# sloisel/MultiGridBarrier.jl

Measured on NVIDIA B200. Metric: mgb_solve DOF*Newton-steps/s (fem2d_P1 ~1.6M DOF, p=1.5), higher is better.
Workload: dtype f64

## Files before the change

multigridbarrier.jl_b200/build.py:

```python
from __future__ import annotations

import os
import shutil
import subprocess
import sys
from concurrent.futures import ThreadPoolExecutor

HERE = os.path.dirname(os.path.abspath(__file__))
CSRC = os.path.join(HERE, "csrc")
OBJ = os.path.join(HERE, "build")
LIB = os.path.join(HERE, "libmgbx.so")
HDR = os.path.join("..", "..", "include", "mgbx.h")
ENGINE = ["engine.hpp", "host_sparse.hpp", "device_common.cuh", "node_barrier.cuh", "pcg2.hpp", HDR]
SOURCES = {
    "mgbx.cu": ["mgbx.cu", "host_amg.hpp"] + ENGINE,
    "setup.cu": ["setup.cu", "setup_kernels.cuh"] + ENGINE,
    "evaluate.cu": ["evaluate.cu", "kernels.cuh", "dense_kernels.cuh"] + ENGINE,
    "linear_solve.cu": ["linear_solve.cu", "solver_kernels.cuh"] + ENGINE,
    "newton.cu": ["newton.cu"] + ENGINE,
    "pcg2.cu": ["pcg2.cu", "pcg2.hpp"],
}
FLAGS = ["-gencode", "arch=compute_100a,code=sm_100a", "-O3", "-DNDEBUG", "-lineinfo", "-std=c++17",
         "-Xcompiler", "-fPIC,-O2,-Wall,-Wno-unused-function"]


def nvcc_path():
    for c in (os.environ.get("NVCC"), shutil.which("nvcc"), "/usr/local/cuda/bin/nvcc"):
        if c and os.path.exists(c):
            return c
    raise RuntimeError("nvcc not found")


def _obj(src):
    return os.path.join(OBJ, os.path.splitext(src)[0] + ".o")


def _stale(src):
    o = _obj(src)
    if not os.path.exists(o):
        return True
    t = os.path.getmtime(o)
    return any(os.path.getmtime(os.path.join(CSRC, d)) > t for d in SOURCES[src])


def needs_build():
    if not os.path.exists(LIB):
        return True
    t = os.path.getmtime(LIB)
    return any(_stale(s) or os.path.getmtime(_obj(s)) > t for s in SOURCES)


def _compile(src, verbose):
    cmd = [nvcc_path()] + FLAGS + (["-Xptxas", "-v"] if verbose else []) + ["-c", os.path.join(CSRC, src), "-o", _obj(src)]
# ... 27 lines not shown
```

multigridbarrier.jl_b200/csrc/device_common.cuh:

```cuda
#pragma once
#include <cuda_runtime.h>
#include <stdint.h>

#include "node_barrier.cuh"

namespace mgbx {

#define MGBX_MAX_OPS 8
constexpr int kRedBlocks = 592;
constexpr int kRedThreads = 256;

struct DevCsr {
  int64_t rows = 0, cols = 0, nnz = 0;
  int64_t *ptr = nullptr;
  int32_t *idx = nullptr;
  double *val = nullptr;
};

__device__ __forceinline__ double warp_sum(double v) {
#pragma unroll
  for (int o = 16; o > 0; o >>= 1) v += __shfl_down_sync(0xffffffffu, v, o);
  return v;
}
__device__ __forceinline__ double warp_max(double v) {
// ... 249 lines not shown
}
__device__ __forceinline__ void fence_proxy_async_smem() { asm volatile("fence.proxy.async.shared::cta;" ::: "memory"); }

struct SellPlan {
  int64_t nout = 0, nslices = 0, nterms = 0;
  int64_t *sptr = nullptr;
  int32_t *cnt = nullptr;
  int32_t *src = nullptr;
  double *w = nullptr;
};

__device__ __forceinline__ int64_t csr_find(const DevCsr &A, int64_t row, int32_t col) {
  int64_t lo = A.ptr[row], hi = A.ptr[row + 1];
  while (lo < hi) {
    const int64_t mid = (lo + hi) >> 1;
    const int32_t c = A.idx[mid];
    if (c < col) lo = mid + 1;
    else if (c > col) hi = mid;
    else return mid;
  }
  return -1;
}

constexpr int kCoarseMaxDense = 128;
inline size_t coarse_inverse_smem(int m) { return sizeof(double) * ((size_t)m * (m + 1) + (size_t)m * (m + 1) / 2 + m); }
inline size_t dense_solve_small_smem(int m) { return sizeof(double) * ((size_t)m * (m + 1) + 2 * (size_t)m); }

constexpr int kGemmBM = 64, kGemmBN = 64, kGemmBK = 16, kGemmLd = kGemmBK + 4;

__device__ __forceinline__ void dmma_m8n8k4(double &d0, double &d1, double a, double b) {
  asm volatile("mma.sync.aligned.m8n8k4.row.col.f64.f64.f64.f64 {%0,%1}, {%2}, {%3}, {%0,%1};" : "+d"(d0), "+d"(d1) : "d"(a), "d"(b));
}

constexpr int kCholNB = 64;
constexpr size_t kCholDiagSmem = sizeof(double) * 2 * kCholNB * (kCholNB + 1);

struct KronCombo {
  const double *Qj, *Qk;
  const double *h;
};
constexpr int kKronMaxCombos = 16;
struct KronWArgs {
  int n1, c2a, c2b, ncombo, K;
  KronCombo c[kKronMaxCombos];
};

struct TopPlanParams {
  DevCsr R;
  DevCsr EincT;
  DevCsr pat;
  const int32_t *rowof;
  int64_t n, N;
  int p, nkept, unit;
  int kept[MGBX_MAX_ND];
  int64_t off[MGBX_MAX_ND + 1];
  int64_t rcol0[MGBX_MAX_ND];
  int pair_of[MGBX_MAX_ND * MGBX_MAX_ND];
};

}
```

multigridbarrier.jl_b200/csrc/engine.hpp:

```cpp
#pragma once
#include <cuda_runtime.h>

#include <chrono>
#include <cmath>
#include <cstdio>
#include <cstring>
#include <functional>
#include <map>
#include <memory>
#include <string>
#include <vector>

#include "host_sparse.hpp"
#include "device_common.cuh"
#include "pcg2.hpp"

namespace mgbx {

#define CK(call)                                                                                      \
  do {                                                                                                \
    cudaError_t e_ = (call);                                                                          \
    if (e_ != cudaSuccess)                                                                            \
      throw std::runtime_error(std::string("CUDA error: ") + cudaGetErrorString(e_) + " at " + __FILE__ + ":" + \
                               std::to_string(__LINE__));                                             \
// ... 182 lines not shown
};

struct EvalOut {
  double y, gnorm;
  bool finite;
  double nonfinite_nodes, lin;
};

}

struct mgbx_handle {
  mgbx::Pool pool;
  mgbx::Amg amg[2];
  std::string err;
  mgbx_config cfg;
  cudaStream_t stream = nullptr;
  bool has_feas = false;
  double *partials = nullptr;
  unsigned int *ticket = nullptr;
  double *dscal = nullptr;
  double *hscal = nullptr;
  mgbx_step_result *res = nullptr;
  int64_t launches = 0;
  int64_t kc_launches[mgbx::KC_COUNT] = {0};
  double kc_ms[mgbx::KC_COUNT] = {0};
  std::vector<cudaEvent_t> ev_free;
  struct Pending {
    int kc;
    cudaEvent_t a, b;
  };
  std::vector<Pending> ev_pending;
  cudaEvent_t ev_cur = nullptr;
  int pcg2_grid = 0;
  double dgemm_flops = 0.0;
  double cur_rtol2 = 1e-22;
  int cur_window = 25;
  int rank = 0, nranks = 1;
  void *comm = nullptr;
  int device = -1;
  std::vector<double> prof_ns;
  std::vector<int64_t> prof_cnt;
  std::vector<unsigned long long> prof_host;
};
namespace mgbx {

struct SolveResult {
  int iters = 0;
  int status = 1;
  double rel = 0.0;
  double erel = 0.0;
};

struct Engine {
  mgbx_handle *h;
  cudaStream_t s;
  explicit Engine(mgbx_handle *hh) : h(hh), s(hh->stream) {}

  void sync() {
    CK(cudaStreamSynchronize(s));
    if (!h->ev_pending.empty()) {
      for (auto &p : h->ev_pending) {
        float ms = 0.f;
        cudaEventElapsedTime(&ms, p.a, p.b);
        if (p.kc >= 0) h->kc_ms[p.kc] += ms;
        else if (h->res) {
          if (p.kc == STAGE_F01) h->res->ms_f01 += ms;
// ... 67 lines not shown
  static int group_for(const DevCsr &A) {
    const double avg = A.rows ? (double)A.nnz / (double)A.rows : 0.0;
    return avg > 48.0 ? 32 : (avg > 6.0 ? 4 : 1);
  }
  void spmv(const DevCsr &A, const double *x, const double *y0, double alpha, double *y, int G = 0);
  void axpby(int64_t m, double a, const double *x, double b, const double *y, double *out);
  void prolong_to_fine(Amg &A, int J, const double *x, const double *zbase, double *zf);
  void restrict_from_fine(Amg &A, int J, const double *gb, double *gJ);
  void dot2_fetch(Amg &A, int J, const double *a, const double *b);
  void maxabs_fetch(int64_t n, const double *v);
  void trial(Amg &A, int J, double sigma);
  void phase1_slack(Amg &A, Amg &F);
  void blockgrad(Amg &A, const ElemParams &E);
  NodeParams node_params(Amg &A, double t);
  ElemParams elem_params(Amg &A);
  bool elem_fused_setup(Amg &A, const NodeParams &NP, int nex, ElemFused &Q, size_t &smem, unsigned int &grid);
  int plap_dim(const Amg &A) const;
  bool plap_setup(Amg &A, int dim, double t, bool use_bw, PlapParams &Q, size_t &smem, unsigned int &grid, bool cond = true);
  EvalOut eval_f01(Amg &A, int J, double t, const double *zbase, const double *x, double *gout, bool use_bw = true);

  System &system_for(Amg &A, int J);
  void assemble(Amg &A, System &S, int J, double t, const double *zbase, const double *x);
  void assemble_unfused(Amg &A, System &S, int J, double t, const double *x);
  void galerkin(System &S, int kend);
  void schur_masks(const Amg &A, const System &S, unsigned &pieces, unsigned &elim) const;
  void assemble_dense(Amg &A, System &S, const NodeParams &P);
  void dgemm_nt(int M, int N, int K, const double *Am, int64_t lda, const double *Bm, int64_t ldb, const double *sc, double *C, int64_t ldc, bool acc, double alpha = 1.0);

  bool precond_fp32(const System &S) const;
  int lambda_power_its(const System &S) const;
  bool use_direct(const System &S, const SysLevel &Lv) const;
  std::vector<int> active_levels(const System &S, int ktop) const;
  void setup_hierarchy(Amg &A, System &S, int ktop);
  void dense_factor(SysLevel &Lv);
  void dense_apply(SysLevel &Lv, const double *b, double *x);
  void direct_solve(SysLevel &Lv, const double *b, double *x);
  SellBuild make_sell(const DevCsr &A, int64_t nthreads);
  void sell_prepare(System &S, int ktop);
  System::Pcg2Dev &pcg2_plan(System &S, int ktop);
  void pcg2_setup_dist(System::Pcg2Dev &D, int nshard);
  SolveResult pcg(System &S, int ktop, const double *b, double *x);
  SolveResult solve_compact(System &S, int ktop, const double *b, double *x);
  SolveResult solve(Amg &A, System &S, int J, const double *g, double *dir);

  struct NewtonOut {
    bool converged;
    int k;
    int status;
    double y, gnorm, inc;
  };
  NewtonOut newton(Amg &A, int J, double t, int maxit, int stop_kind, double lambda_tol, double theta, const mgbx_step_opts &o);
  int step(int which, double t, const mgbx_step_opts &o, mgbx_step_result *r);
  int matched_t(double t_default, double *t_out, double *tstar_out);
};

void solve_kernels_init();
void kron_w_init(size_t smem);

inline bool dense_mode(const Amg &A) { return A.N == 1 && A.p > 64; }
constexpr int kDenseMaxUnknowns = 8192;

template <class F>
bool kron_factor(F M, int r1, int r2, int c1, int c2, std::vector<double> &A, std::vector<double> &B) {
  const int64_t rows = (int64_t)r1 * r2, cols = (int64_t)c1 * c2;
  double best = 0.0;
  int64_t pr = 0, pc = 0;
  for (int64_t r = 0; r < rows; ++r)
    for (int64_t c = 0; c < cols; ++c) {
      const double v = std::fabs(M(r, c));
      if (v > best) {
        best = v;
        pr = r;
        pc = c;
      }
    }
  if (!(best > 0.0) || !std::isfinite(best)) return false;
  const int a0 = (int)(pr / r2), b0 = (int)(pr % r2), g0 = (int)(pc / c2), d0 = (int)(pc % c2);
  A.assign((size_t)r1 * c1, 0.0);
  B.assign((size_t)r2 * c2, 0.0);
  for (int b = 0; b < r2; ++b)
    for (int d = 0; d < c2; ++d) B[(size_t)b * c2 + d] = M((int64_t)a0 * r2 + b, (int64_t)g0 * c2 + d);
  const double piv = B[(size_t)b0 * c2 + d0];
  for (int a = 0; a < r1; ++a)
    for (int g = 0; g < c1; ++g) A[(size_t)a * c1 + g] = M((int64_t)a * r2 + b0, (int64_t)g * c2 + d0) / piv;
  const double tol = 1e-12 * best;
  for (int64_t r = 0; r < rows; ++r)
    for (int64_t c = 0; c < cols; ++c)
      if (std::fabs(M(r, c) - A[(size_t)(r / r2) * c1 + (c / c2)] * B[(size_t)(r % r2) * c2 + (c % c2)]) > tol) return false;
  return true;
// ... 13 lines not shown
```

multigridbarrier.jl_b200/csrc/linear_solve.cu:

```cuda
#include "engine.hpp"
#include "solver_kernels.cuh"

namespace mgbx {

void solve_kernels_init() {
  CK(cudaFuncSetAttribute(k_coarse_inverse, cudaFuncAttributeMaxDynamicSharedMemorySize, (int)coarse_inverse_smem(kCoarseMaxDense)));
  CK(cudaFuncSetAttribute(k_dense_solve_small, cudaFuncAttributeMaxDynamicSharedMemorySize, (int)dense_solve_small_smem(kCoarseMaxDense)));
  CK(cudaFuncSetAttribute(k_chol_diag_inv, cudaFuncAttributeMaxDynamicSharedMemorySize, (int)kCholDiagSmem));
  CK(cudaFuncSetAttribute(k_chol_solve_blocked, cudaFuncAttributeMaxDynamicSharedMemorySize, (int)(sizeof(double) * kDenseMaxUnknowns)));
}

bool Engine::precond_fp32(const System &S) const {
  if (h->cfg.precond_fp32 != 2) return h->cfg.precond_fp32 == 1;
  int64_t tot = 0;
  for (const SysLevel &Lv : S.lev) tot += Lv.A.nnz;
  return tot >= 10000000;
}
int Engine::lambda_power_its(const System &S) const {
  if (h->cfg.lambda_power >= 0) return h->cfg.lambda_power;
  if (S.lev.empty() || S.lev[0].A.rows == 0) return 0;
  return ((double)S.lev[0].A.nnz / (double)S.lev[0].A.rows > 16.0) ? 6 : 0;
}
bool Engine::use_direct(const System &S, const SysLevel &Lv) const {
  return S.dense || Lv.m <= h->cfg.dense_direct_max;
}
std::vector<int> Engine::active_levels(const System &S, int ktop) const {
  const int nlev = (int)S.lev.size();
  const int kend = (S.cut >= 0) ? std::max(S.cut, ktop) : nlev - 1;
  std::vector<int> act;
  for (int k = ktop; k <= kend; ++k) {
    if (k < kend && S.lev[k].T_identity) continue;
    act.push_back(k);
  }
  return act;
}

void Engine::setup_hierarchy(Amg &A, System &S, int ktop) {
  const int nlev = (int)S.lev.size();
  SysLevel &Ltop = S.lev[ktop];
  const bool direct = use_direct(S, Ltop);
  int kend = ktop;
  if (!direct) kend = (S.cut >= 0) ? std::max(S.cut, ktop) : nlev - 1;
  galerkin(S, kend);
  if (direct) {
    if (Ltop.m > kCoarseMaxDense) dense_factor(Ltop);
    return;
  }
  for (int k = ktop; k <= kend; ++k) {
    SysLevel &Lv = S.lev[k];
    CK(cudaMemsetAsync(Lv.lam, 0, sizeof(double), s));
    LAUNCH(KC_VEC, k_l1diag<<<nblk(Lv.m), 256, 0, s>>>(Lv.A, Lv.dinv, Lv.diag, (unsigned long long *)Lv.lam));
    if (precond_fp32(S)) {
      if (!Lv.val32) Lv.val32 = h->pool.alloc<float>(Lv.A.nnz);
      LAUNCH(KC_VEC, k_f64_to_f32<<<nblk(Lv.A.nnz), 256, 0, s>>>(Lv.A.nnz, Lv.A.val, Lv.val32));
    }
  }
  if (S.cut >= 0 && S.cut >= ktop) {
    SysLevel &Lc = S.lev[S.cut];
    const int m = (int)Lc.m;
    if (!Lc.dense_inv) Lc.dense_inv = h->pool.alloc<double>((size_t)m * m);
    LAUNCH(KC_DENSE, k_coarse_inverse<<<1, 1024, coarse_inverse_smem(m), s>>>(Lc.A, Lc.dense_inv));
  }
  sell_prepare(S, ktop);
  if (lambda_power_its(S) > 0) {
    System::Pcg2Dev &D = pcg2_plan(S, ktop);
    if ((int64_t)D.host.nlev * h->pcg2_grid > 3 * (int64_t)kPcg2MaxGrid) throw std::runtime_error("internal: too many levels for the power-iteration kernel");
    LAUNCH(KC_VEC, CK(pcg2_lambda_power(D.dev, h->pcg2_grid, lambda_power_its(S), 1.2, s)));
  }
}

void Engine::dense_factor(SysLevel &Lv) {
  const int m = (int)Lv.m;
  if (m == 0) return;
  const int npan = (m + kCholNB - 1) / kCholNB;
  if (!Lv.dense) {
    Lv.dense = h->pool.alloc<double>((size_t)m * m);
    Lv.dscale = h->pool.alloc<double>(m);
    Lv.dense_inv = h->pool.alloc<double>((size_t)npan * kCholNB * kCholNB);
  }
  zero(Lv.dense, (int64_t)m * m);
  LAUNCH(KC_DENSE, k_dense_scale_diag<<<nblk(m), 256, 0, s>>>(Lv.A, Lv.dscale));
  LAUNCH(KC_DENSE, k_csr_to_dense<<<nblk(m), 256, 0, s>>>(Lv.A, Lv.dscale, Lv.dense));
  for (int p = 0; p < npan; ++p) {
    const int k0 = p * kCholNB, nb = std::min(kCholNB, m - k0), rem = m - k0 - nb;
    double *Li = Lv.dense_inv + (size_t)p * kCholNB * kCholNB;
    LAUNCH(KC_DENSE, k_chol_diag_inv<<<1, 1024, kCholDiagSmem, s>>>(Lv.dense, m, k0, Li));
    if (rem > 0) {
      double *A21 = Lv.dense + (size_t)(k0 + nb) * m + k0;
      dgemm_nt(rem, nb, nb, A21, m, Li, kCholNB, nullptr, A21, m, false);
      dgemm_nt(rem, rem, nb, A21, m, A21, m, nullptr, Lv.dense + (size_t)(k0 + nb) * m + k0 + nb, m, true, -1.0);
    }
  }
}

void Engine::dense_apply(SysLevel &Lv, const double *b, double *x) {
  const int m = (int)Lv.m;
  LAUNCH(KC_DENSE, k_chol_solve_blocked<<<1, 1024, sizeof(double) * m, s>>>(Lv.dense, m, Lv.dense_inv, Lv.dscale, b, x));
}

void Engine::direct_solve(SysLevel &Lv, const double *b, double *x) {
  const bool small = Lv.m <= kCoarseMaxDense;
  auto apply = [&](const double *rhs, double *out) {
    if (small) LAUNCH(KC_DENSE, k_dense_solve_small<<<1, 1024, dense_solve_small_smem((int)Lv.m), s>>>(Lv.A, rhs, out, nullptr));
    else dense_apply(Lv, rhs, out);
  };
  apply(b, x);
  spmv(Lv.A, x, b, -1.0, Lv.r, Lv.spmv_group);
  apply(Lv.r, Lv.x2);
  axpby(Lv.m, 1.0, x, 1.0, Lv.x2, x);
}

SellBuild Engine::make_sell(const DevCsr &A, int64_t nthreads) {
  SellBuild B;
  h->pool.cat = "solve kernel: sliced-ELL level matrices";
  if (A.rows >= INT32_MAX / 2) throw std::runtime_error("persistent solve kernel: a level matrix exceeds 32-bit indexing");
  int lpr = 1;
  const double avg = A.rows ? (double)A.nnz / (double)A.rows : 0.0;
  while (lpr < 32 && A.rows * (int64_t)lpr * 2 <= nthreads && avg / lpr >= 2.0) lpr *= 2;
  const int rps = 32 / lpr;
  const int nsl = (int)((A.rows + rps - 1) / rps);
  B.M.rows = (int)A.rows;
  B.M.lpr = lpr;
  B.M.nslices = nsl;
  B.M.spc = pcg2_slices_per_cta(nsl, std::max(1, h->pcg2_grid));
  if (nsl == 0) return B;
  int *width = tmp_alloc<int>(nsl, s);
  CK(sell_slice_widths(A.rows, lpr, A.ptr, width, s));
  std::vector<int> hw(nsl);
  CK(cudaMemcpyAsync(hw.data(), width, sizeof(int) * nsl, cudaMemcpyDeviceToHost, s));
  CK(cudaStreamSynchronize(s));
  tmp_free(width, s);
  std::vector<int> soff(nsl + 1, 0);
  int64_t tot = 0;
  for (int q = 0; q < nsl; ++q) {
    tot += 32 * (int64_t)hw[q];
    if (tot > INT32_MAX) throw std::runtime_error("persistent solve kernel: sliced-ELL level matrix exceeds 32-bit indexing");
    soff[q + 1] = (int)tot;
// ... 304 lines not shown
```

multigridbarrier.jl_b200/csrc/mgbx.cu:

```cuda
#include <dlfcn.h>

#include <numeric>

#include "engine.hpp"
#include "host_amg.hpp"

using namespace mgbx;

namespace {

thread_local std::string g_last_error;
const char *kKClassNames[KC_COUNT] = {"node_f01", "node_f2", "blockgrad", "blockhess", "csr_gather", "spmv", "spgemm",
                                             "vector", "condense", "dense", "pcg_persistent", "elem_f01", "elem_f2", "dgemm_dmma", "elem_generic_f01", "elem_generic_f2"};

Amg &amg_arg(mgbx_handle *h, int which, const char *prefix = "") {
  if (which < 0 || which > 1 || (which == 1 && !h->has_feas)) throw ArgError(std::string(prefix) + "no such AMG");
  return h->amg[which];
}
Amg &level_arg(mgbx_handle *h, int which, int level) {
  Amg &A = amg_arg(h, which);
  if (level < 0 || level >= A.L) throw ArgError("no such level");
  return A;
}

// ... 117 lines not shown
int mgbx_create(const mgbx_problem *prob, const mgbx_config *cfg, mgbx_handle **out) {
  if (!prob || !out) {
    g_last_error = "mgbx_create: null argument";
    return MGBX_ERR_ARG;
  }
  *out = nullptr;
  mgbx_handle *h = new mgbx_handle();
  if (cfg) h->cfg = *cfg;
  else mgbx_default_config(&h->cfg);
  if (h->cfg.dense_direct_max > kDenseMaxUnknowns) h->cfg.dense_direct_max = kDenseMaxUnknowns;
  if (h->cfg.coarse_max > kCoarseMaxDense) h->cfg.coarse_max = kCoarseMaxDense;
  if (h->cfg.coarse_max < 0) h->cfg.coarse_max = 0;
  h->cur_rtol2 = h->cfg.pcg_rtol * h->cfg.pcg_rtol;
  int rc = guarded(h, [&]() -> int {
    if (h->cfg.persistent != 2) throw ArgError("mgbx_config.persistent must be 2 (the only solve kernel)");
    int ndev = 0;
    cudaError_t e = cudaGetDeviceCount(&ndev);
    if (e != cudaSuccess || ndev == 0)
      throw std::runtime_error("CUDA device required: libmgbx has no CPU fallback (cudaGetDeviceCount: " +
                               std::string(cudaGetErrorString(e)) + ")");
    if (h->cfg.device >= 0) CK(cudaSetDevice(h->cfg.device));
    CK(cudaGetDevice(&h->device));
    CK(cudaStreamCreateWithFlags(&h->stream, cudaStreamNonBlocking));
    h->pool.stream = h->stream;
    {
      int dev = 0;
      CK(cudaGetDevice(&dev));
      cudaMemPool_t mp = nullptr;
      CK(cudaDeviceGetDefaultMemPool(&mp, dev));
      uint64_t keep = UINT64_MAX;
      CK(cudaMemPoolSetAttribute(mp, cudaMemPoolAttrReleaseThreshold, &keep));
      h->pcg2_grid = pcg2_grid(dev);
      if (h->pcg2_grid == 0) throw std::runtime_error("CUDA device cannot run the cooperative solve kernel");
      solve_kernels_init();
    }
    h->partials = h->pool.zeros<double>((size_t)kRedBlocks * 8, h->stream);
    h->ticket = h->pool.zeros<unsigned int>(4, h->stream);
    h->dscal = h->pool.zeros<double>(64, h->stream);
    CK(cudaMallocHost((void **)&h->hscal, sizeof(double) * 64));
    const mgbx_amg &a0 = prob->amg[0];
    create_amg(h, a0, h->amg[0]);
    Amg &A = h->amg[0];
    if (!prob->f_grid || !prob->g_grid) throw ArgError("f_grid / g_grid missing");
    CK(cudaMemcpyAsync(A.f, prob->f_grid, sizeof(double) * A.n * A.nD, cudaMemcpyHostToDevice, h->stream));
    CK(cudaMemcpyAsync(A.z, prob->g_grid, sizeof(double) * A.n * A.nu, cudaMemcpyHostToDevice, h->stream));
    CK(cudaMemcpyAsync(A.zinit, prob->g_grid, sizeof(double) * A.n * A.nu, cudaMemcpyHostToDevice, h->stream));
    if (prob->barrier_weights) A.bw = h->pool.upload<double>(prob->barrier_weights, A.n, h->stream);
    HostTimer tq;
    upload_convex(h, prob->Q, A.n, A.nD, A.cd);
    if (h->cfg.verbose > 0) fprintf(stderr, "[mgbx] convex set scanned + uploaded %.3fs\n", tq.lap());
    if (prob->amg[1].n > 0) attach_feasibility(h, prob->amg[1]);
    CK(cudaStreamSynchronize(h->stream));
    return MGBX_OK;
  });
  if (rc != MGBX_OK) {
    g_last_error = h->err;
    mgbx_destroy(h);
    return rc;
  }
  *out = h;
  return MGBX_OK;
}

static void *g_comm = nullptr;
static int g_comm_rank = -1, g_comm_nranks = 0;
static int g_comm_users = 0;

void mgbx_destroy(mgbx_handle *h) {
  if (!h) return;
  if (h->device >= 0) cudaSetDevice(h->device);
// ... 489 lines not shown
```

multigridbarrier.jl_b200/csrc/pcg2.cu:

```cuda
#include "pcg2.hpp"

#include <math.h>

namespace mgbx {
namespace {

__device__ __forceinline__ double warp_sum2(double v) {
#pragma unroll
  for (int o = 16; o > 0; o >>= 1) v += __shfl_down_sync(0xffffffffu, v, o);
  return v;
}

__device__ __forceinline__ void grid_barrier2(unsigned int *bar) {
  __syncthreads();
  if (threadIdx.x == 0) {
    unsigned int nb = 1;
    if (blockIdx.x == 0) nb = 0x80000000u - (gridDim.x - 1);
    unsigned int old, cur;
    asm volatile("atom.add.release.gpu.u32 %0,[%1],%2;" : "=r"(old) : "l"(bar), "r"(nb) : "memory");
    int spins = 0;
    do {
      asm volatile("ld.acquire.gpu.u32 %0,[%1];" : "=r"(cur) : "l"(bar) : "memory");
      if (++spins > 64) __nanosleep(40);
    } while (((old ^ cur) & 0x80000000u) == 0);
  }
  __syncthreads();
}

enum { PK_FIRST2 = 0, PK_PRE = 1, PK_RESID = 2, PK_RESTRICT = 3, PK_TAIL = 4, PK_PROLONG = 5, PK_POST = 6, PK_DENSE = 7, PK_RZSUM = 8, PK_MATVEC = 9,
       PK_UPDATE = 10, PK_INIT = 11 };
__device__ __forceinline__ void prof_mark(unsigned long long *prof, int tag) {
  if (prof && blockIdx.x == 0 && threadIdx.x == 0) {
    unsigned long long t;
    asm volatile("mov.u64 %0, %%globaltimer;" : "=l"(t));
    const unsigned long long n = prof[0];
    if (n + 1 < (unsigned long long)kPcg2ProfCap) {
      prof[1 + 2 * n] = (unsigned long long)tag;
      prof[2 + 2 * n] = t;
      prof[0] = n + 1;
    }
  }
}

template <bool GRID>
struct Ld {
  static __device__ __forceinline__ int i(const int *p) { return GRID ? __ldg(p) : *p; }
  static __device__ __forceinline__ double m(const double *p) { return GRID ? __ldg(p) : *p; }
  static __device__ __forceinline__ float mf(const float *p) { return GRID ? __ldg(p) : *p; }
  static __device__ __forceinline__ double v(const double *p) { return GRID ? __ldcg(p) : *p; }
};

struct XRt {
  unsigned long long epoch;
  int aborted;
};
__device__ __forceinline__ unsigned long long gtime() {
  unsigned long long t;
  asm volatile("mov.u64 %0, %%globaltimer;" : "=l"(t));
  return t;
// ... 850 lines not shown
```

multigridbarrier.jl_b200/csrc/solver_kernels.cuh:

```cuda
#pragma once

#include "device_common.cuh"

namespace mgbx {

__global__ void __launch_bounds__(256) k_condense_rhs(CondParams P, const double *__restrict__ g, double *Gt) {
  const int64_t i = (int64_t)blockIdx.x * blockDim.x + threadIdx.x;
  if (i >= P.n) return;
  double gE[4], tE[4], Hi[16];
  const int nE = P.nE;
  for (int ev = 0; ev < nE; ++ev) gE[ev] = g[P.Eoff[ev] + i];
  int q = 0;
  for (int a = 0; a < nE; ++a)
    for (int b = a; b < nE; ++b, ++q) {
      const double v = P.hEEinv[i + (int64_t)q * P.n];
      Hi[a * nE + b] = v;
      Hi[b * nE + a] = v;
    }
  for (int ev = 0; ev < nE; ++ev) {
    double s = 0.0;
    for (int ew = 0; ew < nE; ++ew) s += Hi[ev * nE + ew] * gE[ew];
    tE[ev] = s;
  }
  for (int a = 0; a < P.nK; ++a) {
// ... 23 lines not shown
      Hi[b * nE + a] = v;
    }
  for (int ev = 0; ev < nE; ++ev) {
    double s = 0.0;
    for (int ew = 0; ew < nE; ++ew) s += Hi[ev * nE + ew] * rE[ew];
    x[P.Eoff[ev] + i] = s;
  }
}

__global__ void k_pw_init(int64_t m, double *v) {
  const int64_t i = (int64_t)blockIdx.x * blockDim.x + threadIdx.x;
  if (i < m) v[i] = 1.0 + 0.5 * cos(0.7 * (double)i) + ((i & 1) ? 0.25 : -0.25);
}

__global__ void __launch_bounds__(256) k_l1diag(DevCsr A, double *dinv, double *diag, unsigned long long *lam_bits) {
  const int64_t row = (int64_t)blockIdx.x * blockDim.x + threadIdx.x;
  double ratio = 0.0;
  if (row < A.rows) {
    double s = 0.0, d = 0.0;
    for (int64_t k = A.ptr[row]; k < A.ptr[row + 1]; ++k) {
      s += fabs(A.val[k]);
      if (A.idx[k] == row) d = A.val[k];
    }
    dinv[row] = s > 0.0 ? 1.0 / s : 0.0;
    if (diag) diag[row] = d > 0.0 ? 1.0 / d : 0.0;
    if (d > 0.0 && isfinite(s)) ratio = s / d;
  }
  if (lam_bits) {
    ratio = warp_max(ratio);
    if ((threadIdx.x & 31) == 0 && ratio > 0.0) atomicMax(lam_bits, (unsigned long long)__double_as_longlong(ratio));
  }
}

__global__ void k_dense_scale_diag(DevCsr A, double *d) {
  const int64_t row = (int64_t)blockIdx.x * blockDim.x + threadIdx.x;
  if (row >= A.rows) return;
  double dg = 0.0;
  for (int64_t k = A.ptr[row]; k < A.ptr[row + 1]; ++k)
    if (A.idx[k] == row) dg = A.val[k];
  d[row] = dg > 0.0 ? 1.0 / sqrt(dg) : 1.0;
}

__global__ void k_csr_to_dense(DevCsr A, const double *d, double *Ad) {
  const int64_t row = (int64_t)blockIdx.x * blockDim.x + threadIdx.x;
  if (row >= A.rows) return;
  const double di = d[row];
  for (int64_t k = A.ptr[row]; k < A.ptr[row + 1]; ++k) Ad[row * A.rows + A.idx[k]] = A.val[k] * di * d[A.idx[k]];
}

__global__ void __launch_bounds__(256) k_dense_symv(const double *__restrict__ M, int m, const double *__restrict__ x, double *y) {
  const int row = (blockIdx.x * blockDim.x + threadIdx.x) >> 5;
  const int lane = threadIdx.x & 31;
  if (row >= m) return;
  const double *r = M + (size_t)row * m;
  double s = 0.0;
  for (int j = lane; j < m; j += 32) s += r[j] * x[j];
  s = warp_sum(s);
  if (lane == 0) y[row] = s;
}

__global__ void k_f64_to_f32(int64_t n, const double *__restrict__ a, float *__restrict__ out) {
  const int64_t i = (int64_t)blockIdx.x * blockDim.x + threadIdx.x;
  if (i < n) out[i] = (float)a[i];
}

__global__ void __launch_bounds__(1024) k_coarse_inverse(DevCsr A, double *Minv) {
  extern __shared__ double sm[];
  const int m = (int)A.rows;
  const int ld = m + 1;
  double *S = sm;
  double *Li = S + (size_t)m * ld;
  double *d = Li + (size_t)m * (m + 1) / 2;
  const int tid = threadIdx.x, nt = blockDim.x;
  for (int t = tid; t < m * ld; t += nt) S[t] = 0.0;
  __syncthreads();
  for (int row = tid; row < m; row += nt) {
    double dg = 0.0;
    for (int64_t k = A.ptr[row]; k < A.ptr[row + 1]; ++k)
      if (A.idx[k] == row) dg = A.val[k];
    d[row] = dg > 0.0 ? 1.0 / sqrt(dg) : 1.0;
  }
  __syncthreads();
// ... 132 lines not shown
      }
      if (tid == 0) {
        const double t = rhs[k];
        rhs[k] = rhs[pr];
        rhs[pr] = t;
      }
    }
    __syncthreads();
    const double pv = S[k * ld + k];
    for (int i = k + 1 + tid; i < m; i += nt) S[i * ld + k] /= pv;
    __syncthreads();
    const int rem = m - k - 1;
    for (int t = tid; t < rem * rem; t += nt) {
      const int i = k + 1 + t / rem, j = k + 1 + t % rem;
      S[i * ld + j] -= S[i * ld + k] * S[k * ld + j];
    }
    for (int i = k + 1 + tid; i < m; i += nt) rhs[i] -= S[i * ld + k] * rhs[k];
    __syncthreads();
  }
  if (tid < 32) {
    for (int k = m - 1; k >= 0; --k) {
      double sacc = 0.0;
      for (int j = k + 1 + tid; j < m; j += 32) sacc += S[k * ld + j] * rhs[j];
      sacc = warp_sum(sacc);
      if (tid == 0) rhs[k] = (rhs[k] - sacc) / S[k * ld + k];
      __syncwarp();
    }
  }
  __syncthreads();
  for (int i = tid; i < m; i += nt) x[i] = rhs[i];
  if (tid == 0 && info) info[0] = 1;
}

__global__ void __launch_bounds__(1024) k_chol_diag_inv(double *A, int m, int k0, double *Linv) {
  extern __shared__ double chol_sm[];
  double (*L)[kCholNB + 1] = reinterpret_cast<double (*)[kCholNB + 1]>(chol_sm);
  double (*Li)[kCholNB + 1] = reinterpret_cast<double (*)[kCholNB + 1]>(chol_sm + kCholNB * (kCholNB + 1));
  const int nb = min(kCholNB, m - k0);
  const int tid = threadIdx.x, nt = blockDim.x;
  for (int t = tid; t < kCholNB * kCholNB; t += nt) {
    const int i = t / kCholNB, j = t % kCholNB;
    L[i][j] = (i < nb && j <= i) ? A[(size_t)(k0 + i) * m + k0 + j] : 0.0;
    Li[i][j] = 0.0;
  }
  __syncthreads();
  for (int j = 0; j < nb; ++j) {
    if (tid == 0) L[j][j] = sqrt(L[j][j]);
    __syncthreads();
    const double pv = L[j][j];
    for (int i = j + 1 + tid; i < nb; i += nt) L[i][j] /= pv;
    __syncthreads();
    const int rem = nb - j - 1;
    for (int t = tid; t < rem * rem; t += nt) {
      const int i = j + 1 + t / rem, k = j + 1 + t % rem;
      if (k <= i) L[i][k] -= L[i][j] * L[k][j];
    }
    __syncthreads();
  }
  const int lane = tid & 31, wid = tid >> 5, nw = nt >> 5;
  for (int c = wid; c < nb; c += nw) {
    if (lane == 0) Li[c][c] = 1.0 / L[c][c];
    __syncwarp();
    for (int i = c + 1; i < nb; ++i) {
      double sacc = 0.0;
      for (int k = c + lane; k < i; k += 32) sacc += L[i][k] * Li[k][c];
      sacc = warp_sum(sacc);
      if (lane == 0) Li[i][c] = -sacc / L[i][i];
      __syncwarp();
    }
  }
  __syncthreads();
  for (int t = tid; t < kCholNB * kCholNB; t += nt) {
    const int i = t / kCholNB, j = t % kCholNB;
    if (i < nb && j <= i) A[(size_t)(k0 + i) * m + k0 + j] = L[i][j];
    Linv[t] = (i < nb && j < nb) ? Li[i][j] : 0.0;
  }
}

__global__ void __launch_bounds__(1024) k_chol_solve_blocked(const double *__restrict__ A, int m, const double *__restrict__ Linv,
                                                              const double *__restrict__ d, const double *__restrict__ b, double *x) {
  extern __shared__ double v[];
  __shared__ double blk[kCholNB];
  const int tid = threadIdx.x, nt = blockDim.x;
  for (int i = tid; i < m; i += nt) v[i] = b[i] * d[i];
  __syncthreads();
  const int npan = (m + kCholNB - 1) / kCholNB;
  for (int pnl = 0; pnl < npan; ++pnl) {
    const int k0 = pnl * kCholNB, nb = min(kCholNB, m - k0);
    const double *Li = Linv + (size_t)pnl * kCholNB * kCholNB;
    if (tid < nb) {
      double sacc = 0.0;
      for (int j = 0; j <= tid; ++j) sacc += Li[tid * kCholNB + j] * v[k0 + j];
      blk[tid] = sacc;
    }
    __syncthreads();
    if (tid < nb) v[k0 + tid] = blk[tid];
    for (int i = k0 + nb + tid; i < m; i += nt) {
      const double *row = A + (size_t)i * m + k0;
      double sacc = 0.0;
      for (int j = 0; j < nb; ++j) sacc += row[j] * blk[j];
      v[i] -= sacc;
    }
    __syncthreads();
  }
  for (int pnl = npan - 1; pnl >= 0; --pnl) {
    const int k0 = pnl * kCholNB, nb = min(kCholNB, m - k0);
    const double *Li = Linv + (size_t)pnl * kCholNB * kCholNB;
    const int lane = tid & 31, wid = tid >> 5, nw = nt >> 5;
    for (int j = wid; j < nb; j += nw) {
      double sacc = 0.0;
      for (int i = k0 + nb + lane; i < m; i += 32) sacc += A[(size_t)i * m + k0 + j] * v[i];
      sacc = warp_sum(sacc);
      if (lane == 0) blk[j] = v[k0 + j] - sacc;
    }
    __syncthreads();
    if (tid < nb) {
      double sacc = 0.0;
      for (int i = tid; i < nb; ++i) sacc += Li[i * kCholNB + tid] * blk[i];
      v[k0 + tid] = sacc;
    }
    __syncthreads();
  }
  for (int i = tid; i < m; i += nt) x[i] = v[i] * d[i];
}

}
```

Before: 508.9 million.

## Fuse dense Cholesky factor and solve into persistent cooperative kernels with grid barriers

Replaces the per-panel launch sequence for the dense coarse Cholesky (diagonal scaling, CSR-to-dense, per-panel diag inverse plus two DGEMM calls) with one cooperative kernel. It uses grid barriers, parallel panel TRSM across blocks and a DMMA-based trailing SYRK update. The triangular solve, residual SpMV and iterative-refinement second solve are likewise fused into one cooperative kernel with a retuned warp-parallel substitution. The goal is to remove many small launches and serialized single-block work, in exchange for grid-wide spin barriers and a dependence on cooperative launch support.

Result: faster. 541.7 million (median of 6 runs) (+6.5%).

```diff
diff --git a/multigridbarrier.jl_b200/build.py b/multigridbarrier.jl_b200/build.py
--- a/multigridbarrier.jl_b200/build.py
+++ b/multigridbarrier.jl_b200/build.py
@@ -18,7 +18,7 @@
     "evaluate.cu": ["evaluate.cu", "kernels.cuh", "dense_kernels.cuh"] + ENGINE,
     "linear_solve.cu": ["linear_solve.cu", "solver_kernels.cuh"] + ENGINE,
     "newton.cu": ["newton.cu"] + ENGINE,
-    "pcg2.cu": ["pcg2.cu", "pcg2.hpp"],
+    "pcg2.cu": ["pcg2.cu", "pcg2.hpp", "device_common.cuh", "node_barrier.cuh", HDR],
 }
 FLAGS = ["-gencode", "arch=compute_100a,code=sm_100a", "-O3", "-DNDEBUG", "-lineinfo", "-std=c++17",
          "-Xcompiler", "-fPIC,-O2,-Wall,-Wno-unused-function"]
diff --git a/multigridbarrier.jl_b200/csrc/device_common.cuh b/multigridbarrier.jl_b200/csrc/device_common.cuh
--- a/multigridbarrier.jl_b200/csrc/device_common.cuh
+++ b/multigridbarrier.jl_b200/csrc/device_common.cuh
@@ -305,8 +305,37 @@
   asm volatile("mma.sync.aligned.m8n8k4.row.col.f64.f64.f64.f64 {%0,%1}, {%2}, {%3}, {%0,%1};" : "+d"(d0), "+d"(d1) : "d"(a), "d"(b));
 }
 
+__device__ __forceinline__ void grid_barrier2(unsigned int *bar) {
+  __syncthreads();
+  if (threadIdx.x == 0) {
+    unsigned int nb = 1;
+    if (blockIdx.x == 0) nb = 0x80000000u - (gridDim.x - 1);
+    unsigned int old, cur;
+    asm volatile("atom.add.release.gpu.u32 %0,[%1],%2;" : "=r"(old) : "l"(bar), "r"(nb) : "memory");
+    int spins = 0;
+    do {
+      asm volatile("ld.acquire.gpu.u32 %0,[%1];" : "=r"(cur) : "l"(bar) : "memory");
+      if (++spins > 64) __nanosleep(40);
+    } while (((old ^ cur) & 0x80000000u) == 0);
+  }
+  __syncthreads();
+}
+
 constexpr int kCholNB = 64;
-constexpr size_t kCholDiagSmem = sizeof(double) * 2 * kCholNB * (kCholNB + 1);
+constexpr int kCholThreads = 256;
+constexpr int kCholSolveThreads = 1024;
+constexpr int kCholLd = kCholNB + 1;
+constexpr int kCholTileLd = kCholNB + 4;
+constexpr size_t kCholFactorSmem = sizeof(double) * 2 * kCholNB * kCholTileLd;
+inline size_t chol_solve_smem(int m) { return sizeof(double) * ((size_t)m + 32 * kCholNB + kCholNB); }
+struct CholArgs {
+  DevCsr A;
+  double *L;
+  double *d;
+  double *Linv;
+  unsigned int *bar;
+  int m;
+};
 
 struct KronCombo {
   const double *Qj, *Qk;
diff --git a/multigridbarrier.jl_b200/csrc/engine.hpp b/multigridbarrier.jl_b200/csrc/engine.hpp
--- a/multigridbarrier.jl_b200/csrc/engine.hpp
+++ b/multigridbarrier.jl_b200/csrc/engine.hpp
@@ -238,6 +238,8 @@
   std::vector<Pending> ev_pending;
   cudaEvent_t ev_cur = nullptr;
   int pcg2_grid = 0;
+  int chol_grid = 0;
+  unsigned int *chol_bar = nullptr;
   double dgemm_flops = 0.0;
   double cur_rtol2 = 1e-22;
   int cur_window = 25;
@@ -371,8 +373,8 @@
   bool use_direct(const System &S, const SysLevel &Lv) const;
   std::vector<int> active_levels(const System &S, int ktop) const;
   void setup_hierarchy(Amg &A, System &S, int ktop);
+  CholArgs chol_args(SysLevel &Lv);
   void dense_factor(SysLevel &Lv);
-  void dense_apply(SysLevel &Lv, const double *b, double *x);
   void direct_solve(SysLevel &Lv, const double *b, double *x);
   SellBuild make_sell(const DevCsr &A, int64_t nthreads);
   void sell_prepare(System &S, int ktop);
@@ -393,7 +395,7 @@
   int matched_t(double t_default, double *t_out, double *tstar_out);
 };
 
-void solve_kernels_init();
+int solve_kernels_init(int dev);
 void kron_w_init(size_t smem);
 
 inline bool dense_mode(const Amg &A) { return A.N == 1 && A.p > 64; }
diff --git a/multigridbarrier.jl_b200/csrc/linear_solve.cu b/multigridbarrier.jl_b200/csrc/linear_solve.cu
--- a/multigridbarrier.jl_b200/csrc/linear_solve.cu
+++ b/multigridbarrier.jl_b200/csrc/linear_solve.cu
@@ -3,11 +3,17 @@
 
 namespace mgbx {
 
-void solve_kernels_init() {
+int solve_kernels_init(int dev) {
   CK(cudaFuncSetAttribute(k_coarse_inverse, cudaFuncAttributeMaxDynamicSharedMemorySize, (int)coarse_inverse_smem(kCoarseMaxDense)));
   CK(cudaFuncSetAttribute(k_dense_solve_small, cudaFuncAttributeMaxDynamicSharedMemorySize, (int)dense_solve_small_smem(kCoarseMaxDense)));
-  CK(cudaFuncSetAttribute(k_chol_diag_inv, cudaFuncAttributeMaxDynamicSharedMemorySize, (int)kCholDiagSmem));
-  CK(cudaFuncSetAttribute(k_chol_solve_blocked, cudaFuncAttributeMaxDynamicSharedMemorySize, (int)(sizeof(double) * kDenseMaxUnknowns)));
+  CK(cudaFuncSetAttribute(k_chol_factor, cudaFuncAttributeMaxDynamicSharedMemorySize, (int)kCholFactorSmem));
+  CK(cudaFuncSetAttribute(k_chol_solve, cudaFuncAttributeMaxDynamicSharedMemorySize, (int)chol_solve_smem(kDenseMaxUnknowns)));
+  int nsm = 0, coop = 0, per_sm_f = 0, per_sm_s = 0;
+  CK(cudaDeviceGetAttribute(&nsm, cudaDevAttrMultiProcessorCount, dev));
+  CK(cudaDeviceGetAttribute(&coop, cudaDevAttrCooperativeLaunch, dev));
+  CK(cudaOccupancyMaxActiveBlocksPerMultiprocessor(&per_sm_f, k_chol_factor, kCholThreads, kCholFactorSmem));
+  CK(cudaOccupancyMaxActiveBlocksPerMultiprocessor(&per_sm_s, k_chol_solve, kCholSolveThreads, chol_solve_smem(kDenseMaxUnknowns)));
+  return (coop && per_sm_f >= 1 && per_sm_s >= 1) ? nsm : 0;
 }
 
 bool Engine::precond_fp32(const System &S) const {
@@ -69,40 +75,39 @@
   }
 }
 
-void Engine::dense_factor(SysLevel &Lv) {
+CholArgs Engine::chol_args(SysLevel &Lv) {
   const int m = (int)Lv.m;
-  if (m == 0) return;
-  const int npan = (m + kCholNB - 1) / kCholNB;
   if (!Lv.dense) {
     Lv.dense = h->pool.alloc<double>((size_t)m * m);
     Lv.dscale = h->pool.alloc<double>(m);
-    Lv.dense_inv = h->pool.alloc<double>((size_t)npan * kCholNB * kCholNB);
-  }
-  zero(Lv.dense, (int64_t)m * m);
-  LAUNCH(KC_DENSE, k_dense_scale_diag<<<nblk(m), 256, 0, s>>>(Lv.A, Lv.dscale));
-  LAUNCH(KC_DENSE, k_csr_to_dense<<<nblk(m), 256, 0, s>>>(Lv.A, Lv.dscale, Lv.dense));
-  for (int p = 0; p < npan; ++p) {
-    const int k0 = p * kCholNB, nb = std::min(kCholNB, m - k0), rem = m - k0 - nb;
-    double *Li = Lv.dense_inv + (size_t)p * kCholNB * kCholNB;
-    LAUNCH(KC_DENSE, k_chol_diag_inv<<<1, 1024, kCholDiagSmem, s>>>(Lv.dense, m, k0, Li));
-    if (rem > 0) {
-      double *A21 = Lv.dense + (size_t)(k0 + nb) * m + k0;
-      dgemm_nt(rem, nb, nb, A21, m, Li, kCholNB, nullptr, A21, m, false);
-      dgemm_nt(rem, rem, nb, A21, m, A21, m, nullptr, Lv.dense + (size_t)(k0 + nb) * m + k0 + nb, m, true, -1.0);
-    }
-  }
-}
-
-void Engine::dense_apply(SysLevel &Lv, const double *b, double *x) {
-  const int m = (int)Lv.m;
-  LAUNCH(KC_DENSE, k_chol_solve_blocked<<<1, 1024, sizeof(double) * m, s>>>(Lv.dense, m, Lv.dense_inv, Lv.dscale, b, x));
+    Lv.dense_inv = h->pool.alloc<double>((size_t)((m + kCholNB - 1) / kCholNB) * kCholNB * kCholNB);
+  }
+  CholArgs a;
+  a.A = Lv.A;
+  a.L = Lv.dense;
+  a.d = Lv.dscale;
+  a.Linv = Lv.dense_inv;
+  a.bar = h->chol_bar;
+  a.m = m;
+  return a;
+}
+
+void Engine::dense_factor(SysLevel &Lv) {
+  if (Lv.m == 0) return;
+  CholArgs a = chol_args(Lv);
+  void *args[] = {(void *)&a};
+  LAUNCH(KC_DENSE, CK(cudaLaunchCooperativeKernel((const void *)k_chol_factor, dim3(h->chol_grid), dim3(kCholThreads), args, kCholFactorSmem, s)));
 }
 
 void Engine::direct_solve(SysLevel &Lv, const double *b, double *x) {
-  const bool small = Lv.m <= kCoarseMaxDense;
+  if (Lv.m > kCoarseMaxDense) {
+    CholArgs a = chol_args(Lv);
+    void *args[] = {(void *)&a, (void *)&b, (void *)&x, (void *)&Lv.r};
+    LAUNCH(KC_DENSE, CK(cudaLaunchCooperativeKernel((const void *)k_chol_solve, dim3(h->chol_grid), dim3(kCholSolveThreads), args, chol_solve_smem(a.m), s)));
+    return;
+  }
   auto apply = [&](const double *rhs, double *out) {
-    if (small) LAUNCH(KC_DENSE, k_dense_solve_small<<<1, 1024, dense_solve_small_smem((int)Lv.m), s>>>(Lv.A, rhs, out, nullptr));
-    else dense_apply(Lv, rhs, out);
+    LAUNCH(KC_DENSE, k_dense_solve_small<<<1, 1024, dense_solve_small_smem((int)Lv.m), s>>>(Lv.A, rhs, out, nullptr));
   };
   apply(b, x);
   spmv(Lv.A, x, b, -1.0, Lv.r, Lv.spmv_group);
diff --git a/multigridbarrier.jl_b200/csrc/mgbx.cu b/multigridbarrier.jl_b200/csrc/mgbx.cu
--- a/multigridbarrier.jl_b200/csrc/mgbx.cu
+++ b/multigridbarrier.jl_b200/csrc/mgbx.cu
@@ -173,10 +173,12 @@
       CK(cudaMemPoolSetAttribute(mp, cudaMemPoolAttrReleaseThreshold, &keep));
       h->pcg2_grid = pcg2_grid(dev);
       if (h->pcg2_grid == 0) throw std::runtime_error("CUDA device cannot run the cooperative solve kernel");
-      solve_kernels_init();
+      h->chol_grid = solve_kernels_init(dev);
+      if (h->chol_grid < 2) throw std::runtime_error("CUDA device cannot run the cooperative dense Cholesky kernels");
     }
     h->partials = h->pool.zeros<double>((size_t)kRedBlocks * 8, h->stream);
     h->ticket = h->pool.zeros<unsigned int>(4, h->stream);
+    h->chol_bar = h->pool.zeros<unsigned int>(1, h->stream);
     h->dscal = h->pool.zeros<double>(64, h->stream);
     CK(cudaMallocHost((void **)&h->hscal, sizeof(double) * 64));
     const mgbx_amg &a0 = prob->amg[0];
diff --git a/multigridbarrier.jl_b200/csrc/pcg2.cu b/multigridbarrier.jl_b200/csrc/pcg2.cu
--- a/multigridbarrier.jl_b200/csrc/pcg2.cu
+++ b/multigridbarrier.jl_b200/csrc/pcg2.cu
@@ -1,4 +1,5 @@
 #include "pcg2.hpp"
+#include "device_common.cuh"
 
 #include <math.h>
 
@@ -9,22 +10,6 @@
 #pragma unroll
   for (int o = 16; o > 0; o >>= 1) v += __shfl_down_sync(0xffffffffu, v, o);
   return v;
-}
-
-__device__ __forceinline__ void grid_barrier2(unsigned int *bar) {
-  __syncthreads();
-  if (threadIdx.x == 0) {
-    unsigned int nb = 1;
-    if (blockIdx.x == 0) nb = 0x80000000u - (gridDim.x - 1);
-    unsigned int old, cur;
-    asm volatile("atom.add.release.gpu.u32 %0,[%1],%2;" : "=r"(old) : "l"(bar), "r"(nb) : "memory");
-    int spins = 0;
-    do {
-      asm volatile("ld.acquire.gpu.u32 %0,[%1];" : "=r"(cur) : "l"(bar) : "memory");
-      if (++spins > 64) __nanosleep(40);
-    } while (((old ^ cur) & 0x80000000u) == 0);
-  }
-  __syncthreads();
 }
 
 enum { PK_FIRST2 = 0, PK_PRE = 1, PK_RESID = 2, PK_RESTRICT = 3, PK_TAIL = 4, PK_PROLONG = 5, PK_POST = 6, PK_DENSE = 7, PK_RZSUM = 8, PK_MATVEC = 9,
diff --git a/multigridbarrier.jl_b200/csrc/solver_kernels.cuh b/multigridbarrier.jl_b200/csrc/solver_kernels.cuh
--- a/multigridbarrier.jl_b200/csrc/solver_kernels.cuh
+++ b/multigridbarrier.jl_b200/csrc/solver_kernels.cuh
@@ -79,22 +79,6 @@
   }
 }
 
-__global__ void k_dense_scale_diag(DevCsr A, double *d) {
-  const int64_t row = (int64_t)blockIdx.x * blockDim.x + threadIdx.x;
-  if (row >= A.rows) return;
-  double dg = 0.0;
-  for (int64_t k = A.ptr[row]; k < A.ptr[row + 1]; ++k)
-    if (A.idx[k] == row) dg = A.val[k];
-  d[row] = dg > 0.0 ? 1.0 / sqrt(dg) : 1.0;
-}
-
-__global__ void k_csr_to_dense(DevCsr A, const double *d, double *Ad) {
-  const int64_t row = (int64_t)blockIdx.x * blockDim.x + threadIdx.x;
-  if (row >= A.rows) return;
-  const double di = d[row];
-  for (int64_t k = A.ptr[row]; k < A.ptr[row + 1]; ++k) Ad[row * A.rows + A.idx[k]] = A.val[k] * di * d[A.idx[k]];
-}
-
 __global__ void __launch_bounds__(256) k_dense_symv(const double *__restrict__ M, int m, const double *__restrict__ x, double *y) {
   const int row = (blockIdx.x * blockDim.x + threadIdx.x) >> 5;
   const int lane = threadIdx.x & 31;
@@ -293,96 +277,256 @@
   if (tid == 0 && info) info[0] = 1;
 }
 
-__global__ void __launch_bounds__(1024) k_chol_diag_inv(double *A, int m, int k0, double *Linv) {
+template <bool INV>
+__device__ void chol_panel_sweep(double (*P)[kCholLd], int nb, int ext) {
+  constexpr int kRS = kCholThreads / kCholNB;
+  const int c = threadIdx.x % kCholNB, g = threadIdx.x / kCholNB;
+  double (*X)[kCholLd] = P + kCholNB;
+  for (int j = 0; j < nb; ++j) {
+    const double rp = 1.0 / sqrt(P[j][j]);
+    if (c > j) {
+      if (c < nb) {
+        const double lc = P[c][j] * rp;
+        for (int r = c + ((g - c) & (kRS - 1)); r < nb; r += kRS) P[r][c] -= (P[r][j] * rp) * lc;
+        if (!INV)
+          for (int e = g; e < ext; e += kRS) X[e][c] -= (X[e][j] * rp) * lc;
+      }
+    } else if (INV) {
+      const double xj = X[j][c] * rp;
+      for (int i = j + 1 + ((g - j - 1) & (kRS - 1)); i < nb; i += kRS) X[i][c] -= (P[i][j] * rp) * xj;
+    }
+    __syncthreads();
+  }
+}
+
+__global__ void __launch_bounds__(kCholThreads) k_chol_factor(CholArgs ca) {
   extern __shared__ double chol_sm[];
-  double (*L)[kCholNB + 1] = reinterpret_cast<double (*)[kCholNB + 1]>(chol_sm);
-  double (*Li)[kCholNB + 1] = reinterpret_cast<double (*)[kCholNB + 1]>(chol_sm + kCholNB * (kCholNB + 1));
-  const int nb = min(kCholNB, m - k0);
-  const int tid = threadIdx.x, nt = blockDim.x;
-  for (int t = tid; t < kCholNB * kCholNB; t += nt) {
-    const int i = t / kCholNB, j = t % kCholNB;
-    L[i][j] = (i < nb && j <= i) ? A[(size_t)(k0 + i) * m + k0 + j] : 0.0;
-    Li[i][j] = 0.0;
-  }
-  __syncthreads();
-  for (int j = 0; j < nb; ++j) {
-    if (tid == 0) L[j][j] = sqrt(L[j][j]);
-    __syncthreads();
-    const double pv = L[j][j];
-    for (int i = j + 1 + tid; i < nb; i += nt) L[i][j] /= pv;
-    __syncthreads();
-    const int rem = nb - j - 1;
-    for (int t = tid; t < rem * rem; t += nt) {
-      const int i = j + 1 + t / rem, k = j + 1 + t % rem;
-      if (k <= i) L[i][k] -= L[i][j] * L[k][j];
-    }
-    __syncthreads();
-  }
-  const int lane = tid & 31, wid = tid >> 5, nw = nt >> 5;
-  for (int c = wid; c < nb; c += nw) {
-    if (lane == 0) Li[c][c] = 1.0 / L[c][c];
-    __syncwarp();
-    for (int i = c + 1; i < nb; ++i) {
-      double sacc = 0.0;
-      for (int k = c + lane; k < i; k += 32) sacc += L[i][k] * Li[k][c];
-      sacc = warp_sum(sacc);
-      if (lane == 0) Li[i][c] = -sacc / L[i][i];
-      __syncwarp();
-    }
-  }
-  __syncthreads();
-  for (int t = tid; t < kCholNB * kCholNB; t += nt) {
-    const int i = t / kCholNB, j = t % kCholNB;
-    if (i < nb && j <= i) A[(size_t)(k0 + i) * m + k0 + j] = L[i][j];
-    Linv[t] = (i < nb && j < nb) ? Li[i][j] : 0.0;
-  }
-}
-
-__global__ void __launch_bounds__(1024) k_chol_solve_blocked(const double *__restrict__ A, int m, const double *__restrict__ Linv,
-                                                              const double *__restrict__ d, const double *__restrict__ b, double *x) {
-  extern __shared__ double v[];
-  __shared__ double blk[kCholNB];
-  const int tid = threadIdx.x, nt = blockDim.x;
-  for (int i = tid; i < m; i += nt) v[i] = b[i] * d[i];
-  __syncthreads();
+  double (*P)[kCholLd] = reinterpret_cast<double (*)[kCholLd]>(chol_sm);
+  constexpr int kWarps = kCholThreads / 32;
+  const int m = ca.m, tid = threadIdx.x, lane = tid & 31, warp = tid >> 5, G = gridDim.x;
+  for (int row = blockIdx.x * kWarps + warp; row < m; row += G * kWarps) {
+    const int64_t k0 = ca.A.ptr[row];
+    unsigned int last = 0;
+    for (int64_t k = k0 + lane; k < ca.A.ptr[row + 1]; k += 32)
+      if (ca.A.idx[k] == row) last = (unsigned int)(k - k0) + 1;
+    last = __reduce_max_sync(0xffffffffu, last);
+    const double dg = last ? ca.A.val[k0 + last - 1] : 0.0;
+    if (lane == 0) ca.d[row] = dg > 0.0 ? 1.0 / sqrt(dg) : 1.0;
+    for (int j = lane; j <= row; j += 32) ca.L[(size_t)row * m + j] = 0.0;
+  }
+  grid_barrier2(ca.bar);
+  for (int row = blockIdx.x * kWarps + warp; row < m; row += G * kWarps) {
+    const double di = __ldcg(ca.d + row);
+    for (int64_t k = ca.A.ptr[row] + lane; k < ca.A.ptr[row + 1]; k += 32) {
+      const int col = ca.A.idx[k];
+      if (col <= row) ca.L[(size_t)row * m + col] = ca.A.val[k] * di * __ldcg(ca.d + col);
+    }
+  }
+  grid_barrier2(ca.bar);
+
   const int npan = (m + kCholNB - 1) / kCholNB;
-  for (int pnl = 0; pnl < npan; ++pnl) {
-    const int k0 = pnl * kCholNB, nb = min(kCholNB, m - k0);
-    const double *Li = Linv + (size_t)pnl * kCholNB * kCholNB;
+  for (int p = 0; p < npan; ++p) {
+    const int k0 = p * kCholNB, nb = min(kCholNB, m - k0), k1 = k0 + nb, rem = m - k1;
+    auto load_diag = [&]() {
+      for (int t = tid; t < kCholNB * kCholNB; t += kCholThreads) {
+        const int r = t / kCholNB, c = t % kCholNB;
+        P[r][c] = (r < nb && c <= r) ? __ldcg(ca.L + (size_t)(k0 + r) * m + k0 + c) : 0.0;
+      }
+    };
+    auto store_l11 = [&]() {
+      for (int t = tid; t < kCholNB * kCholNB; t += kCholThreads) {
+        const int r = t / kCholNB, c = t % kCholNB;
+        if (r < nb && c <= r) ca.L[(size_t)(k0 + r) * m + k0 + c] = (r == c) ? sqrt(P[r][r]) : P[r][c] * (1.0 / sqrt(P[c][c]));
+      }
+    };
+    if (blockIdx.x == 0) {
+      load_diag();
+      for (int t = tid; t < kCholNB * kCholNB; t += kCholThreads) P[kCholNB + t / kCholNB][t % kCholNB] = (t / kCholNB == t % kCholNB) ? 1.0 : 0.0;
+      __syncthreads();
+      chol_panel_sweep<true>(P, nb, 0);
+      double *Li = ca.Linv + (size_t)p * kCholNB * kCholNB;
+      for (int t = tid; t < kCholNB * kCholNB; t += kCholThreads) {
+        const int r = t / kCholNB, c = t % kCholNB;
+        Li[t] = (r < nb && c <= r) ? P[kCholNB + r][c] * (1.0 / sqrt(P[r][r])) : 0.0;
+      }
+    } else if (rem > 0) {
+      const int workers = G - 1;
+      const int rc = min(kCholNB, (rem + workers - 1) / workers);
+      const int nchunk = (rem + rc - 1) / rc;
+      for (int q = blockIdx.x - 1; q < nchunk; q += workers) {
+        const int r0 = k1 + q * rc, ext = min(rc, m - r0);
+        __syncthreads();
+        load_diag();
+        for (int t = tid; t < ext * kCholNB; t += kCholThreads)
+          P[kCholNB + t / kCholNB][t % kCholNB] = __ldcg(ca.L + (size_t)(r0 + t / kCholNB) * m + k0 + t % kCholNB);
+        __syncthreads();
+        chol_panel_sweep<false>(P, nb, ext);
+        for (int t = tid; t < ext * kCholNB; t += kCholThreads) {
+          const int e = t / kCholNB, c = t % kCholNB;
+          ca.L[(size_t)(r0 + e) * m + k0 + c] = P[kCholNB + e][c] * (1.0 / sqrt(P[c][c]));
+        }
+      }
+    }
+    if (rem == 0) {
+      if (blockIdx.x == 0) store_l11();
+      break;
+    }
+    grid_barrier2(ca.bar);
+    if (blockIdx.x == 0) store_l11();
+    double (*Ti)[kCholTileLd] = reinterpret_cast<double (*)[kCholTileLd]>(chol_sm);
+    double (*Tj)[kCholTileLd] = Ti + kCholNB;
+    const int nt = (rem + kCholNB - 1) / kCholNB, ntiles = nt * (nt + 1) / 2;
+    const int wm = warp >> 2, wn = warp & 3, lr = lane >> 2, lk = lane & 3;
+    for (int t = blockIdx.x; t < ntiles; t += G) {
+      int I = (int)((sqrt(8.0 * t + 1.0) - 1.0) * 0.5);
+      while ((I + 1) * (I + 2) / 2 <= t) ++I;
+      while (I * (I + 1) / 2 > t) --I;
+      const int J = t - I * (I + 1) / 2;
+      const int i0 = k1 + I * kCholNB, j0 = k1 + J * kCholNB;
+      __syncthreads();
+      for (int q = tid; q < kCholNB * kCholNB; q += kCholThreads) {
+        const int r = q / kCholNB, k = q % kCholNB;
+        Ti[r][k] = (i0 + r < m) ? __ldcg(ca.L + (size_t)(i0 + r) * m + k0 + k) : 0.0;
+        if (I != J) Tj[r][k] = (j0 + r < m) ? __ldcg(ca.L + (size_t)(j0 + r) * m + k0 + k) : 0.0;
+      }
+      __syncthreads();
+      double (*B)[kCholTileLd] = (I == J) ? Ti : Tj;
+      double acc[4][2][2];
+#pragma unroll
+      for (int a = 0; a < 4; ++a)
+#pragma unroll
+        for (int b = 0; b < 2; ++b) acc[a][b][0] = acc[a][b][1] = 0.0;
+#pragma unroll
+      for (int k4 = 0; k4 < kCholNB; k4 += 4) {
+        double af[4], bf[2];
+#pragma unroll
+        for (int a = 0; a < 4; ++a) af[a] = Ti[wm * 32 + a * 8 + lr][k4 + lk];
+#pragma unroll
+        for (int b = 0; b < 2; ++b) bf[b] = B[wn * 16 + b * 8 + lr][k4 + lk];
+#pragma unroll
+        for (int a = 0; a < 4; ++a)
+#pragma unroll
+          for (int b = 0; b < 2; ++b) dmma_m8n8k4(acc[a][b][0], acc[a][b][1], af[a], bf[b]);
+      }
+#pragma unroll
+      for (int a = 0; a < 4; ++a)
+#pragma unroll
+        for (int b = 0; b < 2; ++b) {
+          const int i = i0 + wm * 32 + a * 8 + lr, j = j0 + wn * 16 + b * 8 + 2 * lk;
+          if (i >= m) continue;
+          double *cp = ca.L + (size_t)i * m + j;
+          if (j <= i) cp[0] = __ldcg(cp) - acc[a][b][0];
+          if (j + 1 <= i) cp[1] = __ldcg(cp + 1) - acc[a][b][1];
+        }
+    }
+    grid_barrier2(ca.bar);
+  }
+}
+
+__device__ __forceinline__ void chol_tri_solve(const double *__restrict__ L, const double *__restrict__ Linv, int m, double *v, double (*red)[kCholNB], double *blk) {
+  constexpr int kWarps = kCholSolveThreads / 32, kU = 4;
+  const int tid = threadIdx.x, lane = tid & 31, warp = tid >> 5;
+  const int npan = (m + kCholNB - 1) / kCholNB;
+  for (int p = 0; p < npan; ++p) {
+    const int k0 = p * kCholNB, nb = min(kCholNB, m - k0), k1 = k0 + nb;
+    const double *Li = Linv + (size_t)p * kCholNB * kCholNB;
+    {
+      const int r = tid >> 4, s = tid & 15;
+      double acc = 0.0;
+#pragma unroll
+      for (int q = 0; q < 4; ++q) {
+        const int c = s + 16 * q;
+        if (c < nb) acc += __ldg(Li + r * kCholNB + c) * v[k0 + c];
+      }
+#pragma unroll
+      for (int o = 8; o > 0; o >>= 1) acc += __shfl_xor_sync(0xffffffffu, acc, o);
+      if (s == 0) blk[r] = acc;
+    }
+    __syncthreads();
+    if (tid < nb) v[k0 + tid] = blk[tid];
+    if (k1 < m) {
+      const double y0 = blk[lane], y1 = blk[lane + 32];
+      for (int i = k1 + warp; i < m; i += kU * kWarps) {
+        double s[kU];
+#pragma unroll
+        for (int u = 0; u < kU; ++u) {
+          const int iu = i + u * kWarps;
+          const double *row = L + (size_t)iu * m + k0;
+          s[u] = iu < m ? __ldg(row + lane) * y0 + __ldg(row + 32 + lane) * y1 : 0.0;
+        }
+#pragma unroll
+        for (int u = 0; u < kU; ++u) s[u] = warp_sum(s[u]);
+        if (lane == 0)
+#pragma unroll
+          for (int u = 0; u < kU; ++u)
+            if (i + u * kWarps < m) v[i + u * kWarps] -= s[u];
+      }
+    }
+    __syncthreads();
+  }
+  for (int p = npan - 1; p >= 0; --p) {
+    const int k0 = p * kCholNB, nb = min(kCholNB, m - k0), k1 = k0 + nb;
+    const double *Li = Linv + (size_t)p * kCholNB * kCholNB;
+    double s0 = 0.0, s1 = 0.0;
+#pragma unroll 4
+    for (int i = k1 + warp; i < m; i += kWarps) {
+      const double xi = v[i];
+      const double *row = L + (size_t)i * m + k0;
+      s0 += __ldg(row + lane) * xi;
+      s1 += __ldg(row + 32 + lane) * xi;
+    }
+    red[warp][lane] = s0;
+    red[warp][lane + 32] = s1;
+    __syncthreads();
+    if (tid < kCholNB) {
+      double s = 0.0;
+      for (int w = 0; w < kWarps; ++w) s += red[w][tid];
+      blk[tid] = tid < nb ? v[k0 + tid] - s : 0.0;
+    }
+    __syncthreads();
+    {
+      const int c = tid % kCholNB, g = tid / kCholNB;
+      double acc = 0.0;
+#pragma unroll
+      for (int q = 0; q < kCholNB / 16; ++q) acc += __ldg(Li + (g + 16 * q) * kCholNB + c) * blk[g + 16 * q];
+      red[g][c] = acc;
+    }
+    __syncthreads();
     if (tid < nb) {
-      double sacc = 0.0;
-      for (int j = 0; j <= tid; ++j) sacc += Li[tid * kCholNB + j] * v[k0 + j];
-      blk[tid] = sacc;
-    }
-    __syncthreads();
-    if (tid < nb) v[k0 + tid] = blk[tid];
-    for (int i = k0 + nb + tid; i < m; i += nt) {
-      const double *row = A + (size_t)i * m + k0;
-      double sacc = 0.0;
-      for (int j = 0; j < nb; ++j) sacc += row[j] * blk[j];
-      v[i] -= sacc;
-    }
-    __syncthreads();
-  }
-  for (int pnl = npan - 1; pnl >= 0; --pnl) {
-    const int k0 = pnl * kCholNB, nb = min(kCholNB, m - k0);
-    const double *Li = Linv + (size_t)pnl * kCholNB * kCholNB;
-    const int lane = tid & 31, wid = tid >> 5, nw = nt >> 5;
-    for (int j = wid; j < nb; j += nw) {
-      double sacc = 0.0;
-      for (int i = k0 + nb + lane; i < m; i += 32) sacc += A[(size_t)i * m + k0 + j] * v[i];
-      sacc = warp_sum(sacc);
-      if (lane == 0) blk[j] = v[k0 + j] - sacc;
-    }
-    __syncthreads();
-    if (tid < nb) {
-      double sacc = 0.0;
-      for (int i = tid; i < nb; ++i) sacc += Li[i * kCholNB + tid] * blk[i];
-      v[k0 + tid] = sacc;
-    }
-    __syncthreads();
-  }
-  for (int i = tid; i < m; i += nt) x[i] = v[i] * d[i];
-}
-
-}
+      double s = 0.0;
+      for (int g = 0; g < 16; ++g) s += red[g][tid];
+      v[k0 + tid] = s;
+    }
+    __syncthreads();
+  }
+}
+
+__global__ void __launch_bounds__(kCholSolveThreads, 1) k_chol_solve(CholArgs ca, const double *__restrict__ b, double *x, double *r) {
+  extern __shared__ double cs_sm[];
+  constexpr int kWarps = kCholSolveThreads / 32;
+  const int m = ca.m, tid = threadIdx.x, lane = tid & 31, warp = tid >> 5;
+  double *v = cs_sm;
+  double (*red)[kCholNB] = reinterpret_cast<double (*)[kCholNB]>(cs_sm + m);
+  double *blk = cs_sm + m + 32 * kCholNB;
+  if (blockIdx.x == 0) {
+    for (int i = tid; i < m; i += kCholSolveThreads) v[i] = b[i] * ca.d[i];
+    __syncthreads();
+    chol_tri_solve(ca.L, ca.Linv, m, v, red, blk);
+    for (int i = tid; i < m; i += kCholSolveThreads) x[i] = v[i] * ca.d[i];
+  }
+  grid_barrier2(ca.bar);
+  for (int row = blockIdx.x * kWarps + warp; row < m; row += gridDim.x * kWarps) {
+    double s = 0.0;
+    for (int64_t k = ca.A.ptr[row] + lane; k < ca.A.ptr[row + 1]; k += 32) s += ca.A.val[k] * __ldcg(x + ca.A.idx[k]);
+    s = warp_sum(s);
+    if (lane == 0) r[row] = b[row] - s;
+  }
+  grid_barrier2(ca.bar);
+  if (blockIdx.x != 0) return;
+  for (int i = tid; i < m; i += kCholSolveThreads) v[i] = __ldcg(r + i) * ca.d[i];
+  __syncthreads();
+  chol_tri_solve(ca.L, ca.Linv, m, v, red, blk);
+  for (int i = tid; i < m; i += kCholSolveThreads) x[i] += v[i] * ca.d[i];
+}
+
+}
```
